# pytorch/audio

Measured on AMD Instinct MI355X. Metric: audio-sec/sec MelSpectrogram (b=256, 16kHz, n_fft=400, n_mels=80), higher is better.
Workload: dtype f32; 1 GPU; MelSpectrogram n_fft=400 hop=160 n_mels=80, batch=256 x 10 s @16 kHz fp32 per GPU (BASELINE configs[1]); per_gpu_batch=256

## Files before the change

audio_amd/csrc/melspec400.h:

```cpp
#pragma once
#include <type_traits>
#include "hd.h"
#include "stft_generic.h"
#include "resample_mfma.h"

namespace aamd {
namespace m400 {

constexpr int kN = 400;
constexpr int kPad = 200;
constexpr int kFramesPerWave = 6;
#ifndef AAMD_M400_WAVES
#define AAMD_M400_WAVES 12
#define AAMD_M400_MINWAVES 3
#endif
constexpr int kWavesPerBlock = AAMD_M400_WAVES;
constexpr int kTOff[20] = {0, 260, 520, 652, 784, 916, 1444, 1576, 128, 388,
                           2104, 2232, 2364, 1708, 1840, 1048, 1180, 1312, 1972, 2492};
constexpr int kTBufDwords = 2492 + 128;
constexpr int kTRow = 44;
constexpr int kTPair = 20 * kTRow;
constexpr int kLdsDwordsPerWave = 3 * kTPair;
constexpr int kPK = 208;
constexpr int kPPair = 416;
// ... 383 lines not shown
    if (blk >= TREG) {
#pragma unroll
      for (int j = 0; j < 10; ++j) tw[j] = twn[j];
      if (blk < 3) tw_load(blk + 1);
    } else {
#pragma unroll
      for (int j = 0; j < 10; ++j) tw[j] = twr[10 * blk + j];
    }
    float wr[5], wi[5];
#pragma unroll
    for (int j = 0; j < 5; ++j) {
      const int s = 5 * blk + j;
      if (s == 0) {
        wr[j] = yr[0];
        wi[j] = yi[0];
      } else {
        wr[j] = yr[s] * tw[2 * j] - yi[s] * tw[2 * j + 1];
        wi[j] = yr[s] * tw[2 * j + 1] + yi[s] * tw[2 * j];
      }
    }
#if defined(__HIP_DEVICE_COMPILE__)
    if (blk == 0) tr_store5<0>(lds_base, wr, wi);
    else if (blk == 1) tr_store5<5>(lds_base, wr, wi);
    else if (blk == 2) tr_store5<10>(lds_base, wr, wi);
    else tr_store5<15>(lds_base, wr, wi);
#else
    const int l = 20 * c.p + c.pi;
#pragma unroll
    for (int j = 0; j < 5; ++j) {
      lds[kTOff[5 * blk + j] + l] = wr[j];
      lds[kTOff[5 * blk + j] + 64 + l] = wi[j];
    }
#endif
  }
}

template <int H, bool WREG = false, int TREG = 0>
AAMD_HD void phase_a(const LaneConst& c, const float (&X)[Hop<H>::nx], float* lds, const float* winr = nullptr,
                     const float* twr = nullptr) {
  float xr[20], xi[20];
  if (WREG) {
#pragma unroll
    for (int q = 0; q < 20; ++q) { xr[q] = X[q] * winr[q]; xi[q] = X[q + H] * winr[q]; }
  } else {
#pragma unroll
    for (int q4 = 0; q4 < 5; ++q4) {
      const F4 w = *reinterpret_cast<const F4*>(c.win + 4 * q4);
      const float wv[4] = {w.x, w.y, w.z, w.w};
#pragma unroll
      for (int e = 0; e < 4; ++e) {
        const int q = 4 * q4 + e;
        xr[q] = X[q] * wv[e];
        xi[q] = X[q + H] * wv[e];
      }
    }
  }
  phase_a_core<TREG>(c, xr, xi, lds, twr);
}

AAMD_HD void phase_b1_load(const LaneConst& c, const float* lds, float (&vr)[20], float (&vi)[20]) {
  const float* col = lds + c.troff;
#pragma unroll
  for (int j = 0; j < 5; ++j) {
    const F4 r = *reinterpret_cast<const F4*>(col + 4 * j);
    const F4 i = *reinterpret_cast<const F4*>(col + 64 + 4 * j);
    vr[4 * j] = r.x; vr[4 * j + 1] = r.y; vr[4 * j + 2] = r.z; vr[4 * j + 3] = r.w;
    vi[4 * j] = i.x; vi[4 * j + 1] = i.y; vi[4 * j + 2] = i.z; vi[4 * j + 3] = i.w;
  }
}

AAMD_HD void phase_b2_send(const LaneConst& c, const float (&zr)[20], const float (&zi)[20],
                           float (&qr)[10], float (&qi)[10]) {
  const bool c0 = (c.col == 0);
#pragma unroll
  for (int i = 0; i < 10; ++i) {
    const int j = 10 + i;
    const float nr = zr[j], ni = zi[j], rr = zr[(j + 1) % 20], ri = zi[(j + 1) % 20];
    qr[i] = c0 ? rr : nr;
    qi[i] = c0 ? ri : ni;
  }
}

AAMD_HD void phase_b2(const LaneConst& c, const float (&zr)[20], const float (&zi)[20],
                      const float (&xr)[10], const float (&xi)[10], float* lds) {
  if (!c.active) return;
  float* P = lds + kPPair * c.p + 2 * c.col;
#pragma unroll
  for (int u = 0; u < 10; ++u) {
    const float cr = xr[9 - u], ci = xi[9 - u];
    const float ar = zr[u] + cr, ai = zi[u] - ci;
    const float br = zr[u] - cr, bi = zi[u] + ci;
    *reinterpret_cast<F2*>(P + 40 * u) = F2{ar * ar + ai * ai, br * br + bi * bi};
  }
  if (c.col == 0) {
    const float ar = zr[10] + zr[10], bi = zi[10] + zi[10];
    *reinterpret_cast<F2*>(P + 400) = F2{ar * ar, bi * bi};
  }
}

AAMD_HD float spec_pow(float m2, float power) {
  if (power == 2.0f) return m2;
  const float m = sqrt(m2);
  if (power == 1.0f) return m;
  return pow(m, power);
}

AAMD_HD void phase_b2_spec(const LaneConst& c, const float (&zr)[20], const float (&zi)[20],
                           const float (&xr)[10], const float (&xi)[10], float power, int phase, float* lds) {
  if (!c.active) return;
  float* Ra = lds + phase + kSpecBins * 2 * c.p + c.col;
  float* Rb = Ra + kSpecBins;
#pragma unroll
  for (int u = 0; u < 10; ++u) {
    const float cr = xr[9 - u], ci = xi[9 - u];
    const float ar = zr[u] + cr, ai = zi[u] - ci;
    const float br = zr[u] - cr, bi = zi[u] + ci;
    Ra[20 * u] = spec_pow(ar * ar + ai * ai, power);
    Rb[20 * u] = spec_pow(br * br + bi * bi, power);
  }
  if (c.col == 0) {
    const float ar = zr[10] + zr[10], bi = zi[10] + zi[10];
    Ra[200] = spec_pow(ar * ar, power);
    Rb[200] = spec_pow(bi * bi, power);
  }
}

AAMD_HD void phase_b2_spec_complex(const LaneConst& c, const float (&zr)[20], const float (&zi)[20],
                                   const float (&xr)[10], const float (&xi)[10], int half, int phase, float* lds) {
  if (!c.active) return;
  const int fa = 2 * c.p - 3 * half, fb = fa + 1;
  const bool wa = fa >= 0 && fa < 3, wb = fb >= 0 && fb < 3;
  float* Ra = lds + phase + 2 * kSpecBins * fa + 2 * c.col;
  float* Rb = lds + phase + 2 * kSpecBins * fb + 2 * c.col;
#pragma unroll
  for (int u = 0; u < 10; ++u) {
    const float cr = xr[9 - u], ci = xi[9 - u];
    if (wa) { Ra[40 * u] = zr[u] + cr; Ra[40 * u + 1] = zi[u] - ci; }
    if (wb) { Rb[40 * u] = zi[u] + ci; Rb[40 * u + 1] = cr - zr[u]; }
  }
  if (c.col == 0) {
    if (wa) { Ra[400] = zr[10] + zr[10]; Ra[401] = 0.0f; }
    if (wb) { Rb[400] = zi[10] + zi[10]; Rb[401] = 0.0f; }
  }
}

AAMD_HD void store_spec(int lane, const float* lds, float* out, int64_t a0, int n_floats) {
  const int phase = (int)(a0 & 3);
  float* base = out + (a0 - phase);
  const int n_pieces = (phase + n_floats + 3) >> 2;
  for (int j = lane; j < n_pieces; j += 64) {
    const int i0 = 4 * j;
    if (i0 >= phase && i0 + 4 <= phase + n_floats) {
      *reinterpret_cast<F4*>(base + i0) = *reinterpret_cast<const F4*>(lds + i0);
    } else {
      for (int e = 0; e < 4; ++e)
        if (i0 + e >= phase && i0 + e < phase + n_floats) base[i0 + e] = lds[i0 + e];
    }
  }
}

#ifndef AAMD_M400_SPEC_FULL
#define AAMD_M400_SPEC_FULL 1
#endif
AAMD_HD void store_spec_full(int lane, const float* lds, float* out, int64_t a0) {
  constexpr int kN = kFramesPerWave * kSpecBins;
  const int phase = (int)(a0 & 3);
  float* base = out + (a0 - phase);
  const int n_pieces = (phase + kN + 3) >> 2;
  F4 v[5];
#pragma unroll
  for (int u = 0; u < 5; ++u) {
    const int j = lane + 64 * u;
    if (u < 4 || j < n_pieces) v[u] = *reinterpret_cast<const F4*>(lds + 4 * j);
  }
#pragma unroll
  for (int u = 0; u < 5; ++u) {
    const int j = lane + 64 * u, i0 = 4 * j;
    const bool full = i0 >= phase && i0 + 4 <= phase + kN;
    if ((u < 4 || j < n_pieces) && full) *reinterpret_cast<F4*>(base + i0) = v[u];
  }
  if (lane == 0 && phase != 0) {
    const float e[4] = {v[0].x, v[0].y, v[0].z, v[0].w};
#pragma unroll
    for (int k = 1; k < 4; ++k)
      if (k >= phase) base[k] = e[k];
  }
  const int jl = n_pieces - 1, il = 4 * jl;
  if (lane + 256 == jl && il + 4 > phase + kN) {
    const float e[4] = {v[4].x, v[4].y, v[4].z, v[4].w};
#pragma unroll
    for (int k = 0; k < 3; ++k)
      if (il + k < phase + kN) base[il + k] = e[k];
  }
}

AAMD_HD float fast_log10(float x) {
#if defined(__HIP_DEVICE_COMPILE__)
  return __log2f(x) * 0.30102999566398120f;
#else
  return log10(x);
#endif
}
AAMD_HD float epi_plog(float x) {
  const float kE = 2.718281828459045f;
#if defined(__HIP_DEVICE_COMPILE__)
  const float lg = __log2f(x) * 0.69314718055994531f;
#else
  const float lg = log(x);
#endif
  const float t = x > kE ? lg : x;
  return t <= kE ? t / kE : t;
}
AAMD_HD float epi_db(float x, const Epi400& e) {
  return e.multiplier * fast_log10(fmax(x, e.amin)) - e.db_sub;
}

AAMD_HD void phase_b2_pad(int lane, float* lds) {
  constexpr int kTail = kPK - 201;
  if (lane < 3 * kTail) {
    const int p = lane / kTail, j = lane - p * kTail;
    *reinterpret_cast<F2*>(lds + kPPair * p + 2 * (201 + j)) = F2{0.0f, 0.0f};
  }
}

template <int NC>
AAMD_HD void mel_chunks(const float* wt, const float* P, float& sa, float& sb) {
  F4 w[NC], q0[NC], q1[NC];
#pragma unroll
  for (int k = 0; k < NC; ++k) {
    w[k] = *reinterpret_cast<const F4*>(wt + 4 * k);
    q0[k] = *reinterpret_cast<const F4*>(P + 8 * k);
    q1[k] = *reinterpret_cast<const F4*>(P + 8 * k + 4);
  }
#pragma unroll
  for (int k = 0; k < NC; ++k) {
    sa += w[k].x * q0[k].x;
    sb += w[k].x * q0[k].y;
    sa += w[k].y * q0[k].z;
    sb += w[k].y * q0[k].w;
    sa += w[k].z * q1[k].x;
    sb += w[k].z * q1[k].y;
    sa += w[k].w * q1[k].z;
    sb += w[k].w * q1[k].w;
  }
}

template <int NR>
struct MelRegs {
  int nc[NR];
  int pm[NR];
  AAMD_HD int poff(int r) const { return pm[r] & 0xffff; }
  AAMD_HD int mel(int r) const { return pm[r] >> 16; }
};

template <int NR>
AAMD_HD void mel_regs_load(const LaneConst& c, const MelTab& mt, MelRegs<NR>& h) {
#pragma unroll
  for (int r = 0; r < NR; ++r) {
    const bool on = r < mt.n_rounds;
    const int row = r * kMelSlots + c.pi;
#if defined(__HIP_DEVICE_COMPILE__)
    h.nc[r] = on ? __builtin_amdgcn_readfirstlane(mt.rc[r]) : 0;
#else
    h.nc[r] = on ? mt.rc[r] : 0;
#endif
    const int poff = on ? 2 * mt.lo2[row] : 0;
    const int mel = on ? mt.row_mel[row] : -1;
    h.pm[r] = (int)(((unsigned)mel << 16) | (unsigned)poff);
  }
}

AAMD_HD constexpr int sig_chunks(int sig, int r) { return (sig >> (4 * r)) & 15; }
constexpr int kSigHtk80 = 0x4221, kSigSlaney80 = 0x4211;

template <int NR = kMelMaxRounds, int SIG = 0, bool FENCED = false>
AAMD_HD void phase_c(const LaneConst& c, const MelTab& mt, const float* lds,
                     float (&acc_a)[NR], float (&acc_b)[NR], const MelRegs<NR>* h = nullptr) {
  const float* Pp = lds + kPPair * c.p;
  const float* wt0 = mt.w + c.pi * mt.ws;
#pragma unroll
  for (int r = 0; r < NR; ++r) {
    float sa = 0.0f, sb = 0.0f;
#if defined(__HIP_DEVICE_COMPILE__)
    if (FENCED && SIG != 0 && r > 0 && (r & 1) == 0) __builtin_amdgcn_sched_barrier(0);
#endif
    if (SIG != 0 || r < mt.n_rounds) {
      const float* wt = wt0 + r * kMelSlots * mt.ws;
      const float* P = Pp + (h ? h->poff(r) : 2 * mt.lo2[r * kMelSlots + c.pi]);
      const int nc = SIG != 0 ? sig_chunks(SIG, r) : (h ? h->nc[r] : mt.rc[r]);
      switch (nc) {
        case 1: mel_chunks<1>(wt, P, sa, sb); break;
        case 2: mel_chunks<2>(wt, P, sa, sb); break;
        case 3: mel_chunks<3>(wt, P, sa, sb); break;
        case 4: mel_chunks<4>(wt, P, sa, sb); break;
        default:
          for (int k = 0; k < nc; ++k) mel_chunks<1>(wt + 4 * k, P + 8 * k, sa, sb);
      }
    }
    acc_a[r] = sa;
    acc_b[r] = sb;
  }
}

template <int NR = kMelMaxRounds, int SIG = 0>
AAMD_HD void store_direct(const LaneConst& c, const MelTab& mt, const float (&acc_a)[NR],
                          const float (&acc_b)[NR], float* out_row, int64_t t0, int n_frames,
                          const MelRegs<NR>* h = nullptr) {
  const int left = (int)(n_frames - t0);
  const bool va = c.active && 2 * c.p < left, vb = c.active && 2 * c.p + 1 < left;
  float* out_tile = out_row + t0 * (int64_t)mt.n_mels;
  const unsigned oa = 2u * (unsigned)c.p * (unsigned)mt.n_mels;
  if (SIG != 0) {
    if (va) {
#pragma unroll
      for (int r = 0; r < NR; ++r) out_tile[oa + (unsigned)h->mel(r)] = acc_a[r];
    }
    if (vb) {
#pragma unroll
      for (int r = 0; r < NR; ++r) out_tile[oa + (unsigned)mt.n_mels + (unsigned)h->mel(r)] = acc_b[r];
    }
    return;
  }
#pragma unroll
  for (int r = 0; r < NR; ++r) {
    if (r < mt.n_rounds) {
      const int m = h ? h->mel(r) : mt.row_mel[r * kMelSlots + c.pi];
      if (m >= 0) {
        if (va) out_tile[oa + (unsigned)m] = acc_a[r];
        if (vb) out_tile[oa + (unsigned)mt.n_mels + (unsigned)m] = acc_b[r];
      }
    }
  }
}

template <int NR = kMelMaxRounds>
AAMD_HD void store_stage(const LaneConst& c, const MelTab& mt, const float (&acc_a)[NR],
                         const float (&acc_b)[NR], float* lds, const MelRegs<NR>* h = nullptr) {
  if (!c.active) return;
  float* oa = lds + 2 * c.p * mt.n_mels;
#pragma unroll
  for (int r = 0; r < NR; ++r) {
    if (r < mt.n_rounds) {
      const int m = h ? h->mel(r) : mt.row_mel[r * kMelSlots + c.pi];
      if (m >= 0) {
        oa[m] = acc_a[r];
        oa[mt.n_mels + m] = acc_b[r];
      }
    }
  }
}

AAMD_HD void store_wide(int lane, const MelTab& mt, const float* lds, float* out_row, int64_t t0,
                        int n_frames) {
  const int64_t left = n_frames - t0;
  const int n_valid = left < kFramesPerWave ? (int)left : kFramesPerWave;
  const int pieces = n_valid * mt.n_mels / 4;
  float* dst = out_row + t0 * (int64_t)mt.n_mels;
  for (int j = lane; j < pieces; j += 64)
    *reinterpret_cast<F4*>(dst + 4 * j) = *reinterpret_cast<const F4*>(lds + 4 * j);
}

#if defined(__HIPCC__)
__device__ __forceinline__ float vmax_raw(float x, float y) {
  float r;
  asm("v_max_f32 %0, %1, %2" : "=v"(r) : "v"(x), "v"(y));
  return r;
}
__device__ __forceinline__ float vmin_raw(float x, float y) {
  float r;
  asm("v_min_f32 %0, %1, %2" : "=v"(r) : "v"(x), "v"(y));
  return r;
}
__device__ __forceinline__ float vmax3_raw(float x, float y, float z) {
  float r;
  asm("v_max3_f32 %0, %1, %2, %3" : "=v"(r) : "v"(x), "v"(y), "v"(z));
  return r;
}
__device__ __forceinline__ float vmin3_raw(float x, float y, float z) {
  float r;
  asm("v_min3_f32 %0, %1, %2, %3" : "=v"(r) : "v"(x), "v"(y), "v"(z));
  return r;
}
__device__ __forceinline__ void wave_lds_fence() {
  asm volatile("" ::: "memory");
}

__device__ __forceinline__ void exchange_partner(float (&qr)[10], float (&qi)[10], unsigned long long self_mask) {
  unsigned long long saved;
  asm volatile(
      "s_mov_b64 %[sv], exec\n\t"
      "s_andn2_b64 exec, exec, %[m]\n\t"
      "s_nop 4\n\t"
      "v_mov_b32_dpp %0, %0 quad_perm:[1,0,3,2] row_mask:0xf bank_mask:0xf\n\t"
      "v_mov_b32_dpp %1, %1 quad_perm:[1,0,3,2] row_mask:0xf bank_mask:0xf\n\t"
      "v_mov_b32_dpp %2, %2 quad_perm:[1,0,3,2] row_mask:0xf bank_mask:0xf\n\t"
      "v_mov_b32_dpp %3, %3 quad_perm:[1,0,3,2] row_mask:0xf bank_mask:0xf\n\t"
      "v_mov_b32_dpp %4, %4 quad_perm:[1,0,3,2] row_mask:0xf bank_mask:0xf\n\t"
      "v_mov_b32_dpp %5, %5 quad_perm:[1,0,3,2] row_mask:0xf bank_mask:0xf\n\t"
      "v_mov_b32_dpp %6, %6 quad_perm:[1,0,3,2] row_mask:0xf bank_mask:0xf\n\t"
      "v_mov_b32_dpp %7, %7 quad_perm:[1,0,3,2] row_mask:0xf bank_mask:0xf\n\t"
      "v_mov_b32_dpp %8, %8 quad_perm:[1,0,3,2] row_mask:0xf bank_mask:0xf\n\t"
      "v_mov_b32_dpp %9, %9 quad_perm:[1,0,3,2] row_mask:0xf bank_mask:0xf\n\t"
      "v_mov_b32_dpp %10, %10 quad_perm:[1,0,3,2] row_mask:0xf bank_mask:0xf\n\t"
      "v_mov_b32_dpp %11, %11 quad_perm:[1,0,3,2] row_mask:0xf bank_mask:0xf\n\t"
      "v_mov_b32_dpp %12, %12 quad_perm:[1,0,3,2] row_mask:0xf bank_mask:0xf\n\t"
      "v_mov_b32_dpp %13, %13 quad_perm:[1,0,3,2] row_mask:0xf bank_mask:0xf\n\t"
      "v_mov_b32_dpp %14, %14 quad_perm:[1,0,3,2] row_mask:0xf bank_mask:0xf\n\t"
      "v_mov_b32_dpp %15, %15 quad_perm:[1,0,3,2] row_mask:0xf bank_mask:0xf\n\t"
      "v_mov_b32_dpp %16, %16 quad_perm:[1,0,3,2] row_mask:0xf bank_mask:0xf\n\t"
      "v_mov_b32_dpp %17, %17 quad_perm:[1,0,3,2] row_mask:0xf bank_mask:0xf\n\t"
      "v_mov_b32_dpp %18, %18 quad_perm:[1,0,3,2] row_mask:0xf bank_mask:0xf\n\t"
      "v_mov_b32_dpp %19, %19 quad_perm:[1,0,3,2] row_mask:0xf bank_mask:0xf\n\t"
      "s_mov_b64 exec, %[sv]"
      : "+v"(qr[0]), "+v"(qr[1]), "+v"(qr[2]), "+v"(qr[3]), "+v"(qr[4]), "+v"(qr[5]), "+v"(qr[6]), "+v"(qr[7]),
        "+v"(qr[8]), "+v"(qr[9]), "+v"(qi[0]), "+v"(qi[1]), "+v"(qi[2]), "+v"(qi[3]), "+v"(qi[4]), "+v"(qi[5]),
        "+v"(qi[6]), "+v"(qi[7]), "+v"(qi[8]), "+v"(qi[9]), [sv] "=&s"(saved)
      : [m] "s"(self_mask));
}

__device__ __forceinline__ void glds16(const void* gsrc, unsigned lds_dst) {
  asm volatile("s_mov_b32 m0, %1\n\ts_nop 0\n\tglobal_load_lds_dwordx4 %0, off" : : "v"(gsrc), "s"(lds_dst) : "memory", "m0");
}

#ifndef AAMD_M400_DMA_SADDR
#define AAMD_M400_DMA_SADDR 1
#endif
__device__ __forceinline__ void glds16s(const void* sbase, unsigned voff_bytes, unsigned lds_dst) {
  asm volatile("s_mov_b32 m0, %2\n\ts_nop 0\n\tglobal_load_lds_dwordx4 %0, %1" : : "v"(voff_bytes), "s"(sbase), "s"(lds_dst) : "memory", "m0");
}
__device__ __forceinline__ void stage_wait() { asm volatile("s_waitcnt vmcnt(0)" ::: "memory"); }

struct TileInfo {
  int64_t row, t0;
  bool staged;
};

__device__ __forceinline__ void atomic_max_f32(float* addr, float v) {
  if (v >= 0.0f) atomicMax(reinterpret_cast<int*>(addr), __float_as_int(v));
  else atomicMin(reinterpret_cast<unsigned int*>(addr), __float_as_uint(v));
}

__global__ void __launch_bounds__(256) mfcc_frag_build_kernel(const float* __restrict__ dct, int n_mels, int n_mfcc,
                                                              float* __restrict__ frag) {
  uint16_t* fh = reinterpret_cast<uint16_t*>(frag);
  const int n = kMfccMT * kMfccSteps * 64 * 8;
  for (int i = blockIdx.x * blockDim.x + threadIdx.x; i < n; i += gridDim.x * blockDim.x) {
    const int j = i & 7, lane = (i >> 3) & 63, g = i >> 9, s = g % kMfccSteps, t = g / kMfccSteps;
    const float v = mfcc_frag_value(dct, n_mels, n_mfcc, t, s, lane, j);
    const uint16_t hi = rsm::f16_bits(v);
    const uint16_t lo = rsm::f16_bits(v - rsm::f16_value(hi));
    fh[mfcc_frag_piece(t, s, 0, lane) * 8 + j] = hi;
    fh[mfcc_frag_piece(t, s, 1, lane) * 8 + j] = lo;
  }
}

__global__ void __launch_bounds__(256) mel_tab_build_kernel(MelBandsDev mb, float* __restrict__ out) {
  MelTab mt{};
  mel_tab_rounds(threadIdx.x, blockDim.x, mb, out, mt);
  __syncthreads();
  mel_tab_fill(threadIdx.x, blockDim.x, mb, out, mt);
}

template <int LAB, int EPI, int H = 8, typename TIn = float, int NR = kMelMaxRounds, int SIG = 0>
__global__ void __launch_bounds__(64 * kWavesPerBlock, AAMD_M400_MINWAVES)
melspec400_kernel(const TIn* __restrict__ wav, const float* __restrict__ window,
                  const float* __restrict__ tw400, MelBandsDev mb, float* __restrict__ out,
                  int64_t rows, int64_t length, int64_t row_stride, int n_frames, float scale,
                  int tiles_per_row, int64_t n_tiles, int tiles_per_block, int in_aligned,
                  int out_wide, Epi400 epi) {
  extern __shared__ __attribute__((aligned(16))) float smem400[];
  unsigned fix_base = 0, fix_cnt = 0;
#if defined(AAMD_LAB) && defined(AAMD_MFCC_FIXUP_RETURNS)
  if (EPI == EPI400_MFCC && epi.fixup != 0) return;
#endif
  if (EPI == EPI400_MFCC && epi.fixup != 0) {
    int* const cnt = reinterpret_cast<int*>(smem400);
    if (threadIdx.x == 0) *cnt = 0;
    __syncthreads();
    const unsigned nt = (unsigned)n_tiles, nbk = gridDim.x, b = blockIdx.x;
    const unsigned n_cand = b < nt ? (nt - b + nbk - 1u) / nbk : 0u;
    fix_base = b * (nt / nbk) + (b < nt % nbk ? b : nt % nbk);
    for (unsigned k0 = 0; k0 < n_cand; k0 += blockDim.x) {
      const unsigned k = k0 + threadIdx.x;
      bool hit = false;
      unsigned t = 0;
      if (k < n_cand) {
        t = b + k * nbk;
        const unsigned row = t / (unsigned)tiles_per_row;
        hit = epi.tile_min[t] < epi.group_max[row / epi.rows_per_group] - epi.top_db;
      }
      const unsigned long long m = __ballot(hit);
      int slot = 0;
      if ((threadIdx.x & 63) == 0 && m)
        slot = __hip_atomic_fetch_add(cnt, __popcll(m), __ATOMIC_RELAXED, __HIP_MEMORY_SCOPE_WORKGROUP);
      slot = __builtin_amdgcn_readfirstlane(slot);
      if (hit) epi.fix_list[fix_base + slot + __popcll(m & ((1ull << (threadIdx.x & 63)) - 1ull))] = (int)t;
    }
    __syncthreads();
    fix_cnt = (unsigned)__builtin_amdgcn_readfirstlane(*cnt);
    if (fix_cnt == 0) return;
    if (threadIdx.x == 0) atomicAdd(epi.fix_count, (int)fix_cnt);
    __syncthreads();
  }
  if (EPI == EPI400_MFCC && epi.fixup == 0 && epi.fix_count != nullptr && !(LAB & (1048576 | 8388608)) && blockIdx.x == 0 &&
      threadIdx.x == 0)
    *epi.fix_count = 0;
  const int elab = (LAB & 524288) ? epi.lab : 0;
  const int lane = threadIdx.x & 63;
  const int wave = __builtin_amdgcn_readfirstlane(threadIdx.x >> 6);
#ifdef AAMD_M400_PRIO
  {
    const int pr = AAMD_M400_PRIO == 1 ? (wave >> 2) : AAMD_M400_PRIO == 2 ? 2 - (wave >> 2) : (wave >> 2) == 0 ? 1 : 0;
    if (pr == 1) __builtin_amdgcn_s_setprio(1);
    else if (pr == 2) __builtin_amdgcn_s_setprio(2);
  }
#endif
  long long lab_t0 = 0;
  if (LAB & 1024) lab_t0 = wall_clock64();
  if ((LAB & 1048576) && lane == 0) {
    long long* rec = reinterpret_cast<long long*>(epi.fix_count);
    const int w = blockIdx.x * kWavesPerBlock + wave;
    rec[4 * w] = (long long)clock64();
    rec[4 * w + 1] = wall_clock64();
  }
  using HC = Hop<H>;
  constexpr int kHop = HC::hop;
  float* lds = smem400 + wave * HC::lds_dwords;
  const unsigned s_addr = (unsigned)(uintptr_t)(lds + kSOff);

  float* const_tab = smem400 + kWavesPerBlock * HC::lds_dwords;
  const_tab_build(threadIdx.x, blockDim.x, window, tw400, scale, const_tab);
  MelTab mt{};
  const int tab_dwords = (EPI != EPI400_SPEC) ? mel_tab_dwords(mb.n_mels, mb.max_width) : 0;
  int* queue = reinterpret_cast<int*>(const_tab + kConstDwords + tab_dwords);
  constexpr bool kIoWave = (LAB & 16777216) != 0;
  constexpr int kNio = kIoWave ? ((LAB & 67108864) ? 2 : 1) : 0;
  if (threadIdx.x == 0) *queue = kWavesPerBlock - kNio;
  float* frag_lds = const_tab + kConstDwords + tab_dwords + 4;
  constexpr bool kFragLds = (H != 10);
  if (EPI == EPI400_MFCC && (epi.frag_in_lds != 0) != kFragLds) __builtin_trap();
  if (EPI == EPI400_MFCC && kFragLds)
    for (int i = threadIdx.x; i < kMfccFragFloats; i += blockDim.x) frag_lds[i] = epi.dct_frag[i];
  if (EPI != EPI400_SPEC && mb.table400 != nullptr) {
    float* dst = const_tab + kConstDwords;
    for (int i = threadIdx.x; i < tab_dwords; i += blockDim.x) dst[i] = mb.table400[i];
    mel_tab_layout(mb, dst, mt);
    __syncthreads();
  } else {
    if (EPI != EPI400_SPEC) mel_tab_rounds(threadIdx.x, blockDim.x, mb, const_tab + kConstDwords, mt);
    __syncthreads();
    if (EPI != EPI400_SPEC) mel_tab_fill(threadIdx.x, blockDim.x, mb, const_tab + kConstDwords, mt);
    __syncthreads();
  }

  long long lab_t1 = 0;
  if (LAB & 1024) lab_t1 = wall_clock64();
  LaneConst c;
  lane_init(lane, const_tab, c);
  constexpr bool kWinRegs = (EPI != EPI400_MFCC || H != 10) && (((LAB & 8192) != 0) || !(LAB & 262144));
  float winr[20], twr[40];
  if (kWinRegs) {
#pragma unroll
    for (int q = 0; q < 20; ++q) winr[q] = c.win[q];
  }
#ifndef AAMD_M400_TWREG
#define AAMD_M400_TWREG 3
#endif
#ifndef AAMD_M400_TWREG_DB
#define AAMD_M400_TWREG_DB 1
#endif
#ifndef AAMD_M400_TWREG_MFCC
#define AAMD_M400_TWREG_MFCC 2
#endif
  constexpr bool kPlain = H == 8 && std::is_same<TIn, float>::value && LAB == 0;
  constexpr int kTwRegBatches = (LAB & 16384) ? 4
                                : (SIG != 0 && EPI == EPI400_MEL) ? AAMD_M400_TWREG
                                : !kPlain ? 0
                                : EPI == EPI400_SPEC ? 2
                                : (EPI == EPI400_MEL && SIG == 0) ? (NR <= 4 ? 1 : 3)
                                : (EPI == EPI400_MFCC && NR <= 4) ? AAMD_M400_TWREG_MFCC
                                : (EPI == EPI400_MEL_DB && NR <= 4) ? AAMD_M400_TWREG_DB : 0;
  if (kTwRegBatches > 0) {
#pragma unroll
    for (int q = 0; q < 10 * kTwRegBatches; ++q) twr[q] = c.tw[q];
  }
  constexpr bool kHoist = NR <= 4;
  MelRegs<NR> mregs;
  const MelRegs<NR>* mh = nullptr;
  if (EPI != EPI400_SPEC && kHoist) {
    mel_regs_load<NR>(c, mt, mregs);
    mh = &mregs;
  }
  if (SIG != 0) {
    static_assert(SIG == 0 || NR == 4, "filterbank signatures are 4 rounds of 20 mels");
    const int sig_rt = mregs.nc[0] | (mregs.nc[1 % NR] << 4) | (mregs.nc[2 % NR] << 8) | (mregs.nc[3 % NR] << 12);
    if (mt.n_rounds != NR || mt.n_mels != kMelSlots * NR || sig_rt != SIG) __builtin_trap();
  }
  if (EPI == EPI400_MFCC && (mt.n_rounds != NR || mt.n_mels != kMelSlots * NR)) __builtin_trap();
  float nrm_mean[NR], nrm_inv[NR];
  if (EPI == EPI400_MEL_NORM) {
#pragma unroll
    for (int r = 0; r < NR; ++r) {
      const int m = r < mt.n_rounds ? mt.row_mel[r * kMelSlots + c.pi] : -1;
      nrm_mean[r] = m >= 0 ? epi.mean[m] : 0.0f;
      nrm_inv[r] = m >= 0 ? epi.invstd[m] : 0.0f;
    }
  }
  const unsigned long long self_mask = __ballot((c.col == 0) || (c.col == 10));
  using SG = Stage<H, TIn>;
  static_assert(SG::ok, "no staging layout for this hop / input type");
  int spiece[SG::ndma];
#pragma unroll
  for (int k = 0; k < SG::ndma; ++k) spiece[k] = SG::spp * stage_src_piece<H, TIn>(64 * k + lane);

  const int nb = gridDim.x;
  int lb = blockIdx.x;
  if ((nb & 7) == 0) lb = (blockIdx.x & 7) * (nb >> 3) + (blockIdx.x >> 3);
  unsigned blk_first = (unsigned)lb * (unsigned)tiles_per_block;
  unsigned blk_count = 0;
  if (blk_first < (unsigned)n_tiles) {
    blk_count = (unsigned)n_tiles - blk_first;
    if (blk_count > (unsigned)tiles_per_block) blk_count = (unsigned)tiles_per_block;
  }
  if (EPI == EPI400_MFCC && epi.fixup != 0) {
    blk_first = 0;
    blk_count = fix_cnt;
  }
  auto claim = [&]() {
    int v = 0;
    if (lane == 0) v = __hip_atomic_fetch_add(queue, 1, __ATOMIC_RELAXED, __HIP_MEMORY_SCOPE_WORKGROUP);
    return (unsigned)__builtin_amdgcn_readfirstlane(v);
  };
#if AAMD_M400_POOLS
#define AAMD_M400_POOLED (AAMD_M400_POOLS && (LAB == 0) && epi.pool != nullptr && !(EPI == EPI400_MFCC && epi.fixup != 0))
  if (AAMD_M400_POOLED && blk_count > (unsigned)(tiles_per_block - epi.pool_p)) blk_count = (unsigned)(tiles_per_block - epi.pool_p);
  unsigned pool_ticket = 0;
  auto pool_request = [&]() {
    int lbo = (int)(blk_first / (unsigned)tiles_per_block);
    asm volatile("" : "+s"(lbo));
    unsigned* const ctr = epi.pool + (lbo % pool_count(nb)) * kPoolStride;
    if (lane == 0) pool_ticket = __hip_atomic_fetch_add(ctr, 1u, __ATOMIC_RELAXED, __HIP_MEMORY_SCOPE_AGENT);
  };
  auto pool_take = [&]() {
    int lbo = (int)(blk_first / (unsigned)tiles_per_block);
    asm volatile("" : "+s"(lbo));
    const int np = pool_count(nb), pid = lbo % np, mem = pool_members(nb, np, pid);
    for (;;) {
      const unsigned v = (unsigned)__builtin_amdgcn_readfirstlane((int)pool_ticket);
      if (v + 1u == (unsigned)(mem * (epi.pool_p + kWavesPerBlock)) && lane == 0)
        __hip_atomic_store(epi.pool + pid * kPoolStride, 0u, __ATOMIC_RELAXED, __HIP_MEMORY_SCOPE_AGENT);
      bool exhausted;
      const unsigned t = pool_tile(np, epi.pool_p, tiles_per_block, (unsigned)n_tiles, pid, mem, v, exhausted);
      if (t != kNoTile) return t - blk_first;
      if (exhausted) return 0x80000000u;
      pool_request();
    }
  };
  constexpr unsigned kBadIdx = 0x80000000u, kPendIdx = 0x80000001u;
#define AAMD_M400_IDX_OK(I) ((((I) ^ 0x80000000u)) > 1u)
#define AAMD_M400_LOCAL(I) ((I) < blk_count ? (I) : kBadIdx)
#else
#define AAMD_M400_IDX_OK(I) ((I) < blk_count)
#define AAMD_M400_LOCAL(I) (I)
#endif
  constexpr unsigned kLabChunk = 8;
  unsigned* gq = reinterpret_cast<unsigned*>(epi.group_max);
  int g_pending = 0;
  unsigned g_base = 0, g_pos = 0;
  auto g_request = [&]() {
    if (lane == 0) g_pending = (int)__hip_atomic_fetch_add(gq, 1u, __ATOMIC_RELAXED, __HIP_MEMORY_SCOPE_AGENT);
  };
  if (LAB & 131072) {
    blk_count = (unsigned)n_tiles;
    g_request();
    g_base = (unsigned)__builtin_amdgcn_readfirstlane(g_pending) * kLabChunk;
    g_request();
  }
  auto g_next = [&]() {
    if (++g_pos < kLabChunk) return g_base + g_pos;
    g_base = (unsigned)__builtin_amdgcn_readfirstlane(g_pending) * kLabChunk;
    g_pos = 0;
    g_request();
    return g_base;
  };

  auto tile_info = [&](unsigned idx) {
    TileInfo ti;
    unsigned t = ((LAB & 131072) ? 0u : blk_first) + idx;
    if (EPI == EPI400_MFCC && epi.fixup != 0)
      t = idx < blk_count ? (unsigned)__hip_atomic_load(epi.fix_list + fix_base + idx, __ATOMIC_RELAXED, __HIP_MEMORY_SCOPE_AGENT) : 0u;
    const unsigned row = t / (unsigned)tiles_per_row;
    ti.row = row;
    ti.t0 = (int64_t)(t - row * (unsigned)tiles_per_row) * kFramesPerWave;
    ti.staged = AAMD_M400_IDX_OK(idx) && in_aligned && (ti.t0 * kHop - kPad >= 0) &&
                ((ti.t0 + kFramesPerWave - 1) * kHop + (kN - kPad) <= length) &&
                (ti.t0 + kFramesPerWave <= n_frames);
    return ti;
  };
  auto stage_issue = [&](const TileInfo& ti) {
    const TIn* src = wav + (ti.row / InTraits<TIn>::chans) * row_stride + (ti.t0 * kHop - kPad);
    if (LAB & 32) src = wav + 6 * kHop;
#pragma unroll
    for (int k = 0; k < SG::ndma; ++k)
      if (!(LAB & 64) || k == 0) {
#if AAMD_M400_DMA_SADDR
        glds16s(src, (unsigned)spiece[k] * (unsigned)sizeof(TIn), s_addr + 1024 * k);
#else
        glds16(src + spiece[k], s_addr + 1024 * k);
#endif
      }
  };

  float wmax = -INFINITY;
  int64_t wgroup = -1, wrow = -1;
  constexpr bool kDb = (EPI == EPI400_MEL_DB) || (EPI == EPI400_MFCC);
  const bool fix = (EPI == EPI400_MFCC) && epi.fixup != 0;
  auto flush_max = [&]() {
    if (kDb && !fix && epi.group_max != nullptr && wgroup >= 0) {
      float m = wmax;
#pragma unroll
      for (int off = 32; off > 0; off >>= 1) m = fmaxf(m, __shfl_xor(m, off, 64));
      if (lane == 0) atomic_max_f32(epi.group_max + wgroup, m);
    }
    wmax = -INFINITY;
  };

  if (kIoWave && wave >= kWavesPerBlock - kNio) {
    constexpr unsigned D = 8;
    constexpr bool kFetchOnly = (LAB & 134217728) != 0;
    if (!(LAB & 33554432)) {
      const unsigned n_mine = (blk_count + (unsigned)kNio - 1u - (unsigned)(wave - (kWavesPerBlock - kNio))) / (unsigned)kNio;
      for (unsigned i = 0; i < n_mine + D; ++i) {
        const unsigned t = i * (unsigned)kNio + (unsigned)(wave - (kWavesPerBlock - kNio));
        if (i < n_mine) {
          const TileInfo ti = tile_info(AAMD_M400_LOCAL(t));
          const unsigned dst = (unsigned)(uintptr_t)(smem400 + (t % (unsigned)kWavesPerBlock) * HC::lds_dwords + kSOff);
          if (ti.staged) {
            const TIn* src = wav + (ti.row / InTraits<TIn>::chans) * row_stride + (ti.t0 * kHop - kPad);
#pragma unroll
            for (int k = 0; k < SG::ndma; ++k) glds16(src + spiece[k], dst + 1024 * k);
          }
        }
        if (i >= D) {
          if (kFetchOnly) {
            asm volatile("s_waitcnt vmcnt(40)" ::: "memory");
          } else {
            asm volatile("s_waitcnt vmcnt(56)" ::: "memory");
            const unsigned told = t - D * (unsigned)kNio;
            const TileInfo to = tile_info(AAMD_M400_LOCAL(told));
            const float* stg = smem400 + (told % (unsigned)kWavesPerBlock) * HC::lds_dwords;
            store_wide(lane, mt, stg, out + to.row * (int64_t)n_frames * (int64_t)mb.n_mels, to.t0, n_frames);
          }
        }
      }
    }
    blk_count = 0;
  }
  unsigned cur_idx = (LAB & 131072) ? g_base : (unsigned)wave;
#if AAMD_M400_POOLS
  if (cur_idx >= blk_count) cur_idx = kBadIdx;
  if (AAMD_M400_POOLED && cur_idx == kBadIdx) {
    pool_request();
    cur_idx = pool_take();
  }
#endif
  TileInfo cur = tile_info(cur_idx);
  if (LAB & 128) {
    const int k = (wave + 6 * lb) % 3;
    for (int i = 0; i < k; ++i) __builtin_amdgcn_s_sleep(112);
  }
  if (LAB & 2048) {
    const int k = 4 * (wave & 3) + (wave >> 2) % 3;
    for (int i = 0; i < (k % 12); ++i) __builtin_amdgcn_s_sleep(17);
  }
  if (LAB & 4096) {
    const int k = 4 * ((wave >> 2) % 3) + (wave & 3);
    for (int i = 0; i < k; ++i) __builtin_amdgcn_s_sleep(17);
  }
  float Xn[HC::nx];
  auto gload = [&](const TileInfo& ti) {
    const TIn* src = wav + (ti.row / InTraits<TIn>::chans) * row_stride + (ti.t0 * kHop - kPad) + (HC::pair_stride * c.p + c.pi);
#pragma unroll
    for (int q = 0; q < HC::nx; ++q) Xn[q] = InTraits<TIn>::get(src + 20 * q, (int)(ti.row % InTraits<TIn>::chans));
  };
  if (LAB & 32768) {
#pragma unroll
    for (int q = 0; q < HC::nx; ++q) Xn[q] = 0.0f;
    if (cur.staged) gload(cur);
  } else if (cur.staged && !(LAB & 8) && !fix) {
    stage_issue(cur);
  }

  long long ph_acc[6] = {0, 0, 0, 0, 0, 0}, ph_t = 0;
  int ph_tiles = 0;
#define AAMD_M400_STAMP(K)                                  \
  if (LAB & 8388608) {                                      \
    const long long now_ = (long long)clock64();            \
    ph_acc[K] += now_ - ph_t;                               \
    ph_t = now_;                                            \
  }
  using mfcc_f32x4 = __attribute__((ext_vector_type(4))) float;
  mfcc_f32x4 cf[kMfccMT];
  const int mfcc_elab = (LAB & 524288) ? epi.lab : 0;
  auto mfcc_finish = [&](int64_t row, int64_t t0) {
#pragma unroll
    for (int t = 0; t < kMfccMT; ++t)
#pragma unroll
      for (int i = 0; i < 4; ++i) {
        cf[t][i] += __int_as_float(__builtin_amdgcn_mov_dpp(__float_as_int(cf[t][i]), 0x128, 0xf, 0xf, true));
        asm volatile("" : "+v"(cf[t][i]));
      }
    const int64_t left64 = n_frames - t0;
    const int left = left64 < kFramesPerWave ? (int)left64 : kFramesPerWave;
    if (!(LAB & 2) && !(mfcc_elab & 8) && (lane & 15) < left) {
      float* otile = out + (row * (int64_t)n_frames + t0) * (int64_t)epi.n_mfcc;
      const unsigned ooff = (unsigned)(lane & 15) * (unsigned)epi.n_mfcc + 4u * (unsigned)(lane >> 4);
#pragma unroll
      for (int t = 0; t < kMfccMT; ++t) {
        const int k0 = 16 * t + 4 * (lane >> 4);
        if (k0 < epi.n_mfcc) *reinterpret_cast<F4*>(otile + (ooff + 16u * (unsigned)t)) = F4{cf[t][0], cf[t][1], cf[t][2], cf[t][3]};
      }
    }
  };
  while (AAMD_M400_IDX_OK(cur_idx)) {
    if (LAB & 8388608) { ph_t = (long long)clock64(); ++ph_tiles; }
#if AAMD_M400_POOLS
    unsigned nxt_idx = (LAB & 131072) ? g_next() : claim();
    if (nxt_idx >= blk_count) nxt_idx = AAMD_M400_POOLED ? kPendIdx : kBadIdx;
#else
    const unsigned nxt_idx = (LAB & 131072) ? g_next() : claim();
#endif
    TileInfo nxt = tile_info(nxt_idx);
    float fix_cut = -INFINITY;
    if (fix) {
      fix_cut = epi.group_max[cur.row / epi.rows_per_group] - epi.top_db;
      if (cur.staged) stage_issue(cur);
    }

    float X[HC::nx];
    if ((LAB & 32768) && cur.staged) {
#pragma unroll
      for (int q = 0; q < HC::nx; ++q) X[q] = Xn[q];
    } else if (cur.staged) {
      if (!(LAB & 1)) stage_wait();
      if (LAB & 256) {
#pragma unroll
        for (int q = 0; q < HC::nx; ++q) X[q] = (float)(q + lane) * scale;
      } else {
        gather_lds<H, TIn>(c, reinterpret_cast<const TIn*>(lds + kSOff), X, (int)(cur.row % InTraits<TIn>::chans));
      }
    } else {
      gather_global<H, TIn>(c, wav + (cur.row / InTraits<TIn>::chans) * row_stride, length, cur.t0, n_frames, X,
                            (int)(cur.row % InTraits<TIn>::chans));
    }
#if AAMD_M400_POOLS
    if (nxt_idx == kPendIdx) pool_request();
#endif
    phase_a<H, kWinRegs, kTwRegBatches>(c, X, lds, winr, twr);
    if ((LAB & 32768) && nxt.staged) gload(nxt);
    wave_lds_fence();
    AAMD_M400_STAMP(0)
    float vr[20], vi[20], zr[20], zi[20], qr[10], qi[10];
    phase_b1_load(c, lds, vr, vi);
    if (!(LAB & 32768)) {
      asm volatile("s_waitcnt lgkmcnt(0)" ::: "memory");
      AAMD_M400_STAMP(1)
#if AAMD_M400_POOLS
      if (nxt_idx == kPendIdx) {
        nxt_idx = pool_take();
        nxt = tile_info(nxt_idx);
      }
#endif
      if (nxt.staged && !(LAB & 8) && !fix) stage_issue(nxt);
    }
    if (LAB & 16) { wave_lds_fence(); cur = nxt; cur_idx = nxt_idx; continue; }
    dft20(vr, vi, zr, zi);
    phase_b2_send(c, zr, zi, qr, qi);
    exchange_partner(qr, qi, self_mask);
    wave_lds_fence();
    AAMD_M400_STAMP(2)
    if (EPI == EPI400_SPEC) {
      const int64_t left = n_frames - cur.t0;
      const int n_valid = left < kFramesPerWave ? (int)left : kFramesPerWave;
      if (epi.power > 0.0f) {
        const int64_t a0 = (cur.row * n_frames + cur.t0) * (int64_t)kSpecBins;
        phase_b2_spec(c, zr, zi, qr, qi, epi.power, (int)(a0 & 3), lds);
        wave_lds_fence();
        if (!(LAB & 2)) {
          if (AAMD_M400_SPEC_FULL && n_valid == kFramesPerWave) store_spec_full(lane, lds, out, a0);
          else store_spec(lane, lds, out, a0, n_valid * kSpecBins);
        }
        wave_lds_fence();
      } else {
#pragma unroll
        for (int half = 0; half < 2; ++half) {
          const int64_t a0 = (cur.row * n_frames + cur.t0 + 3 * half) * (int64_t)(2 * kSpecBins);
          const int nv = n_valid - 3 * half < 3 ? n_valid - 3 * half : 3;
          phase_b2_spec_complex(c, zr, zi, qr, qi, half, (int)(a0 & 3), lds);
          wave_lds_fence();
          if (!(LAB & 2) && nv > 0) store_spec(lane, lds, out, a0, nv * 2 * kSpecBins);
          wave_lds_fence();
        }
      }
      cur = nxt;
      cur_idx = nxt_idx;
      continue;
    }
    phase_b2(c, zr, zi, qr, qi, lds);
    phase_b2_pad(lane, lds);
    wave_lds_fence();
    AAMD_M400_STAMP(3)
    float acc_a[NR], acc_b[NR];
    if (LAB & 4) { wave_lds_fence(); cur = nxt; cur_idx = nxt_idx; continue; }
    phase_c<NR, SIG, EPI == EPI400_MFCC>(c, mt, lds, acc_a, acc_b, mh);
    if (LAB & 8388608) { asm volatile("" : "+v"(acc_a[0]), "+v"(acc_b[NR - 1])); }
    AAMD_M400_STAMP(4)
    if (kDb) {
      if (cur.row != wrow) {
        wrow = cur.row;
        const int64_t g = cur.row / epi.rows_per_group;
        if (g != wgroup) {
          flush_max();
          wgroup = g;
        }
      }
      const bool va_ok = cur.t0 + 2 * c.p < n_frames, vb_ok = cur.t0 + 2 * c.p + 1 < n_frames;
      float tmin = INFINITY;
      if (EPI == EPI400_MFCC) {
        const float db_c1 = epi.multiplier * 0.30102999566398120f;
#pragma unroll
        for (int r = 0; r < NR; ++r) {
          acc_a[r] = __builtin_fmaf(__log2f(vmax_raw(acc_a[r], epi.amin)), db_c1, -epi.db_sub);
          acc_b[r] = __builtin_fmaf(__log2f(vmax_raw(acc_b[r], epi.amin)), db_c1, -epi.db_sub);
        }
        if (cur.t0 + kFramesPerWave <= n_frames) {
#pragma unroll
          for (int r = 0; r < NR; ++r) {
            wmax = vmax3_raw(wmax, acc_a[r], acc_b[r]);
            tmin = vmin3_raw(tmin, acc_a[r], acc_b[r]);
          }
        } else {
#pragma unroll
          for (int r = 0; r < NR; ++r) {
            wmax = fmaxf(wmax, fmaxf(va_ok ? acc_a[r] : -INFINITY, vb_ok ? acc_b[r] : -INFINITY));
            tmin = fminf(tmin, fminf(va_ok ? acc_a[r] : INFINITY, vb_ok ? acc_b[r] : INFINITY));
          }
        }
        if (fix) {
#pragma unroll
          for (int r = 0; r < NR; ++r) {
            acc_a[r] = vmax_raw(acc_a[r], fix_cut);
            acc_b[r] = vmax_raw(acc_b[r], fix_cut);
          }
        }
      } else {
        const bool interior = cur.t0 + kFramesPerWave <= n_frames;
#pragma unroll
        for (int r = 0; r < NR; ++r) {
          if (r < mt.n_rounds) {
            acc_a[r] = epi.multiplier * fast_log10(vmax_raw(acc_a[r], epi.amin)) - epi.db_sub;
            acc_b[r] = epi.multiplier * fast_log10(vmax_raw(acc_b[r], epi.amin)) - epi.db_sub;
            if (interior) wmax = vmax3_raw(wmax, acc_a[r], acc_b[r]);
            else wmax = fmaxf(wmax, fmaxf(va_ok ? acc_a[r] : -INFINITY, vb_ok ? acc_b[r] : -INFINITY));
          }
        }
      }
      if (EPI == EPI400_MFCC && !fix && !(elab & 4)) {
        asm volatile(
            "s_nop 1\n\t"
            "v_min_f32_dpp %0, %0, %0 row_shr:1 row_mask:0xf bank_mask:0xf\n\ts_nop 1\n\t"
            "v_min_f32_dpp %0, %0, %0 row_shr:2 row_mask:0xf bank_mask:0xf\n\ts_nop 1\n\t"
            "v_min_f32_dpp %0, %0, %0 row_shr:4 row_mask:0xf bank_mask:0xf\n\ts_nop 1\n\t"
            "v_min_f32_dpp %0, %0, %0 row_shr:8 row_mask:0xf bank_mask:0xf\n\ts_nop 1\n\t"
            "v_min_f32_dpp %0, %0, %0 row_bcast:15 row_mask:0xa bank_mask:0xf\n\ts_nop 1\n\t"
            "v_min_f32_dpp %0, %0, %0 row_bcast:31 row_mask:0xc bank_mask:0xf"
            : "+v"(tmin));
        if (lane == 63) epi.tile_min[blk_first + cur_idx] = tmin;
      }
    }
    if (EPI == EPI400_MFCC) {
      using f32x4 = __attribute__((ext_vector_type(4))) float;
      using h8 = __attribute__((ext_vector_type(8))) _Float16;
      using h4 = __attribute__((ext_vector_type(4))) _Float16;
      using u32x4 = __attribute__((ext_vector_type(4))) uint32_t;
      using u32x2 = __attribute__((ext_vector_type(2))) uint32_t;
      wave_lds_fence();
      {
        uint16_t* hs = reinterpret_cast<uint16_t*>(lds);
        uint16_t* ls = hs + kMfccPlaneHalves;
#pragma unroll
        for (int r = 0; r < NR; ++r) {
          const int m = mh ? mh->mel(r) : mt.row_mel[r * kMelSlots + c.pi];
          const float va = acc_a[r] * kMfccYScale, vb = acc_b[r] * kMfccYScale;
          const _Float16 ha = (_Float16)va, hb = (_Float16)vb;
          const _Float16 la = (_Float16)(va - (float)ha), lb = (_Float16)(vb - (float)hb);
          hs[2 * c.p * kMfccMels + m] = __builtin_bit_cast(uint16_t, ha);
          ls[2 * c.p * kMfccMels + m] = __builtin_bit_cast(uint16_t, la);
          hs[(2 * c.p + 1) * kMfccMels + m] = __builtin_bit_cast(uint16_t, hb);
          ls[(2 * c.p + 1) * kMfccMels + m] = __builtin_bit_cast(uint16_t, lb);
        }
      }
      wave_lds_fence();
#pragma unroll
      for (int t = 0; t < kMfccMT; ++t) cf[t] = f32x4{0.0f, 0.0f, 0.0f, 0.0f};
      auto product = [&](const u32x4* __restrict__ ftab) {
        const uint16_t* hs = reinterpret_cast<const uint16_t*>(lds);
        u32x4 a0[kMfccMT][2];
        auto frag_load = [&](int sidx) {
#pragma unroll
          for (int t = 0; t < kMfccMT; ++t)
#pragma unroll
            for (int hl = 0; hl < 2; ++hl) {
              a0[t][hl] = u32x4{0x3c003c00u, 0x3c003c00u, 0x3c003c00u, 0x3c003c00u};
              if (!(elab & 1)) a0[t][hl] = ftab[mfcc_frag_piece(t, sidx, hl, lane)];
            }
        };
#pragma unroll
        for (int sidx = 0; sidx < 2; ++sidx) {
          const h8 bb = __builtin_bit_cast(h8, *reinterpret_cast<const u32x4*>(hs + mfcc_b_index(lane, sidx)));
          frag_load(sidx);
#pragma unroll
          for (int t = 0; t < kMfccMT; ++t)
            cf[t] = __builtin_amdgcn_mfma_f32_16x16x32_f16(__builtin_bit_cast(h8, a0[t][1]), bb, cf[t], 0, 0, 0);
#pragma unroll
          for (int t = 0; t < kMfccMT; ++t)
            cf[t] = __builtin_amdgcn_mfma_f32_16x16x32_f16(__builtin_bit_cast(h8, a0[t][0]), bb, cf[t], 0, 0, 0);
        }
        {
          frag_load(2);
          const h4 bb = __builtin_bit_cast(h4, *reinterpret_cast<const u32x2*>(hs + mfcc_b_index(lane, 2)));
#define AAMD_A4(T, HL) __builtin_bit_cast(h4, u32x2{a0[T][HL][0], a0[T][HL][1]})
#pragma unroll
          for (int t = 0; t < kMfccMT; ++t) cf[t] = __builtin_amdgcn_mfma_f32_16x16x16f16(AAMD_A4(t, 1), bb, cf[t], 0, 0, 0);
#pragma unroll
          for (int t = 0; t < kMfccMT; ++t) cf[t] = __builtin_amdgcn_mfma_f32_16x16x16f16(AAMD_A4(t, 0), bb, cf[t], 0, 0, 0);
#undef AAMD_A4
        }
      };
      if (!(elab & 2)) {
        if (kFragLds) product(reinterpret_cast<const u32x4*>(frag_lds));
        else product(reinterpret_cast<const u32x4*>(epi.dct_frag));
      }
      if (!(elab & 2)) mfcc_finish(cur.row, cur.t0);
      wave_lds_fence();
      cur = nxt;
      cur_idx = nxt_idx;
      continue;
    }
    if (EPI == EPI400_MEL_NORM) {
#pragma unroll
      for (int r = 0; r < NR; ++r) {
        if (r < mt.n_rounds) {
          acc_a[r] = (epi_plog(acc_a[r] * epi.gain) - nrm_mean[r]) * nrm_inv[r];
          acc_b[r] = (epi_plog(acc_b[r] * epi.gain) - nrm_mean[r]) * nrm_inv[r];
        }
      }
    }
    float* out_row = out + cur.row * (EPI == EPI400_MEL_NORM ? epi.out_frames : (int64_t)n_frames) * (int64_t)mb.n_mels;
    if (LAB & 4194304) out_row = out + (int64_t)(wave + kWavesPerBlock * (blockIdx.x & 63)) * 6 * mb.n_mels - cur.t0 * (int64_t)mb.n_mels;
    if (out_wide) {
      wave_lds_fence();
      store_stage<NR>(c, mt, acc_a, acc_b, lds, mh);
      wave_lds_fence();
      if (!(LAB & 2)) store_wide(lane, mt, lds, out_row, cur.t0, n_frames);
    } else {
      if (!(LAB & 2)) store_direct<NR, SIG>(c, mt, acc_a, acc_b, out_row, cur.t0, n_frames, mh);
    }
    wave_lds_fence();
    AAMD_M400_STAMP(5)
    cur = nxt;
    cur_idx = nxt_idx;
  }
#undef AAMD_M400_STAMP
  if ((LAB & 8388608) && lane == 0) {
    long long* rec = reinterpret_cast<long long*>(epi.fix_count) + 4 * 12 * 256 + 8 * (blockIdx.x * kWavesPerBlock + wave);
#pragma unroll
    for (int k = 0; k < 6; ++k) rec[k] = ph_acc[k];
    rec[6] = ph_tiles;
  }
  if (kDb && !fix && epi.group_max != nullptr) {
    float m = wmax;
#pragma unroll
    for (int off = 32; off > 0; off >>= 1) m = fmaxf(m, __shfl_xor(m, off, 64));
    if (lane == 0) {
      reinterpret_cast<int*>(lds)[0] = (int)wgroup;
      lds[1] = m;
    }
    __syncthreads();
    if (threadIdx.x == 0) {
      int g_run = -1;
      float m_run = -INFINITY;
      for (int w = 0; w < kWavesPerBlock; ++w) {
        const int gw = reinterpret_cast<const int*>(smem400 + w * HC::lds_dwords)[0];
        const float mw = smem400[w * HC::lds_dwords + 1];
        if (gw != g_run) {
          if (g_run >= 0) atomic_max_f32(epi.group_max + g_run, m_run);
          g_run = gw;
          m_run = mw;
        } else {
          m_run = fmaxf(m_run, mw);
        }
      }
      if (g_run >= 0) atomic_max_f32(epi.group_max + g_run, m_run);
    }
  }
  if ((LAB & 1048576) && lane == 0) {
    long long* rec = reinterpret_cast<long long*>(epi.fix_count);
    const int w = blockIdx.x * kWavesPerBlock + wave;
    rec[4 * w + 2] = (long long)clock64();
    rec[4 * w + 3] = wall_clock64();
  }
  if ((LAB & 1024) && lane == 0) {
    long long* rec = reinterpret_cast<long long*>(const_cast<float*>(tw400) + 1024);
    const int w = blockIdx.x * kWavesPerBlock + wave;
    rec[3 * w] = lab_t0;
    rec[3 * w + 1] = lab_t1;
    rec[3 * w + 2] = wall_clock64();
  }
}
#endif

}
}
```

Measured before the change: 37.47 million audio-sec/sec.

## Cut per-tile scalar address math: carry tile offsets, saddr stores, LDS queue claim

Precomputes per-tile input/output offsets in TileInfo and advances them incrementally from the previous tile instead of recomputing divisions and 64-bit multiplies. The staged-tile test is simplified to a precomputed tile-index range. Mel output stores use global_store_dword with a scalar base and immediate offsets, with a fast path for full tiles. The tile-queue claim uses an inline ds_add_rtn in place of the HIP atomic. This targets the integer and address overhead in the persistent tile loop. It adds inline asm and carry logic that must stay consistent with the tile indexing.

```diff
diff --git a/audio_amd/csrc/melspec400.h b/audio_amd/csrc/melspec400.h
--- a/audio_amd/csrc/melspec400.h
+++ b/audio_amd/csrc/melspec400.h
@@ -709,6 +709,15 @@
   }
 }
 
+template <int OFF>
+AAMD_HD void store_f32_saddr(float v, char* base, unsigned voff) {
+#if defined(__HIP_DEVICE_COMPILE__)
+  asm volatile("global_store_dword %0, %1, %2 offset:%3" : : "v"(voff), "v"(v), "s"(base), "i"(OFF) : "memory");
+#else
+  *reinterpret_cast<float*>(base + (size_t)voff + OFF) = v;
+#endif
+}
+
 template <int NR = kMelMaxRounds, int SIG = 0>
 AAMD_HD void store_direct(const LaneConst& c, const MelTab& mt, const float (&acc_a)[NR],
                           const float (&acc_b)[NR], float* out_row, int64_t t0, int n_frames,
@@ -718,13 +727,27 @@
   float* out_tile = out_row + t0 * (int64_t)mt.n_mels;
   const unsigned oa = 2u * (unsigned)c.p * (unsigned)mt.n_mels;
   if (SIG != 0) {
+    constexpr unsigned nm = kMelSlots * NR;
+    char* const ob = reinterpret_cast<char*>(out_row + t0 * (int64_t)nm);
+    unsigned bo[NR];
+#pragma unroll
+    for (int r = 0; r < NR; ++r) bo[r] = 4u * (2u * (unsigned)c.p * nm + (unsigned)h->mel(r));
+    if (left >= kFramesPerWave) {
+      if (c.active) {
+#pragma unroll
+        for (int r = 0; r < NR; ++r) store_f32_saddr<0>(acc_a[r], ob, bo[r]);
+#pragma unroll
+        for (int r = 0; r < NR; ++r) store_f32_saddr<4 * (int)nm>(acc_b[r], ob, bo[r]);
+      }
+      return;
+    }
     if (va) {
 #pragma unroll
-      for (int r = 0; r < NR; ++r) out_tile[oa + (unsigned)h->mel(r)] = acc_a[r];
+      for (int r = 0; r < NR; ++r) store_f32_saddr<0>(acc_a[r], ob, bo[r]);
     }
     if (vb) {
 #pragma unroll
-      for (int r = 0; r < NR; ++r) out_tile[oa + (unsigned)mt.n_mels + (unsigned)h->mel(r)] = acc_b[r];
+      for (int r = 0; r < NR; ++r) store_f32_saddr<4 * (int)nm>(acc_b[r], ob, bo[r]);
     }
     return;
   }
@@ -838,8 +861,12 @@
 __device__ __forceinline__ void stage_wait() { asm volatile("s_waitcnt vmcnt(0)" ::: "memory"); }
 
 struct TileInfo {
-  int64_t row, t0;
+  int64_t row;
+  int t0;
   bool staged;
+  unsigned tin;
+  int64_t in_off;
+  int64_t out_off;
 };
 
 __device__ __forceinline__ void atomic_max_f32(float* addr, float v) {
@@ -1033,9 +1060,11 @@
     blk_first = 0;
     blk_count = fix_cnt;
   }
+  const unsigned queue_addr = (unsigned)(uintptr_t)queue;
   auto claim = [&]() {
     int v = 0;
-    if (lane == 0) v = __hip_atomic_fetch_add(queue, 1, __ATOMIC_RELAXED, __HIP_MEMORY_SCOPE_WORKGROUP);
+    if (lane == 0)
+      asm volatile("ds_add_rtn_u32 %0, %1, %2\n\ts_waitcnt lgkmcnt(0)" : "=v"(v) : "v"(queue_addr), "v"(1) : "memory");
     return (unsigned)__builtin_amdgcn_readfirstlane(v);
   };
 #if AAMD_M400_POOLS
@@ -1091,6 +1120,21 @@
     return g_base;
   };
 
+  static_assert(kFramesPerWave * kHop >= kPad, "tile 1 starts inside the clip");
+  unsigned tin_hi = 0;
+  if (in_aligned && length >= kN - kPad) {
+    int64_t last = (length - (kN - kPad)) / kHop - (kFramesPerWave - 1);
+    if (last > (int64_t)n_frames - kFramesPerWave) last = (int64_t)n_frames - kFramesPerWave;
+    if (last >= kFramesPerWave) tin_hi = (unsigned)(last / kFramesPerWave);
+  }
+  const int64_t out_row_elems =
+      EPI == EPI400_SPEC   ? (int64_t)n_frames * (epi.power > 0.0f ? kSpecBins : 2 * kSpecBins)
+      : EPI == EPI400_MFCC ? (int64_t)n_frames * epi.n_mfcc
+                           : (EPI == EPI400_MEL_NORM ? epi.out_frames : (int64_t)n_frames) * (int64_t)mb.n_mels;
+  auto tile_fill = [&](TileInfo& ti, unsigned idx) {
+    ti.t0 = (int)ti.tin * kFramesPerWave;
+    ti.staged = AAMD_M400_IDX_OK(idx) && ti.tin - 1u < tin_hi;
+  };
   auto tile_info = [&](unsigned idx) {
     TileInfo ti;
     unsigned t = ((LAB & 131072) ? 0u : blk_first) + idx;
@@ -1098,14 +1142,33 @@
       t = idx < blk_count ? (unsigned)__hip_atomic_load(epi.fix_list + fix_base + idx, __ATOMIC_RELAXED, __HIP_MEMORY_SCOPE_AGENT) : 0u;
     const unsigned row = t / (unsigned)tiles_per_row;
     ti.row = row;
-    ti.t0 = (int64_t)(t - row * (unsigned)tiles_per_row) * kFramesPerWave;
-    ti.staged = AAMD_M400_IDX_OK(idx) && in_aligned && (ti.t0 * kHop - kPad >= 0) &&
-                ((ti.t0 + kFramesPerWave - 1) * kHop + (kN - kPad) <= length) &&
-                (ti.t0 + kFramesPerWave <= n_frames);
+    ti.tin = t - row * (unsigned)tiles_per_row;
+    ti.in_off = (ti.row / InTraits<TIn>::chans) * row_stride;
+    ti.out_off = ti.row * out_row_elems;
+    tile_fill(ti, idx);
+    return ti;
+  };
+  constexpr bool kCarry = !(LAB & (131072 | 16777216)) && !AAMD_M400_POOLS && EPI != EPI400_MFCC && InTraits<TIn>::chans == 1;
+  constexpr unsigned kCarryMinTiles = 16;
+  auto tile_next = [&](const TileInfo& from, unsigned from_idx, unsigned idx) {
+    if (!kCarry || (unsigned)tiles_per_row < kCarryMinTiles) return tile_info(idx);
+    TileInfo ti = from;
+    if (!(AAMD_M400_IDX_OK(idx))) {
+      ti.staged = false;
+      return ti;
+    }
+    ti.tin = from.tin + (idx - from_idx);
+    while (ti.tin >= (unsigned)tiles_per_row) {
+      ti.tin -= (unsigned)tiles_per_row;
+      ti.row += 1;
+      ti.in_off += row_stride;
+      ti.out_off += out_row_elems;
+    }
+    tile_fill(ti, idx);
     return ti;
   };
   auto stage_issue = [&](const TileInfo& ti) {
-    const TIn* src = wav + (ti.row / InTraits<TIn>::chans) * row_stride + (ti.t0 * kHop - kPad);
+    const TIn* src = wav + ti.in_off + ((int64_t)ti.t0 * kHop - kPad);
     if (LAB & 32) src = wav + 6 * kHop;
 #pragma unroll
     for (int k = 0; k < SG::ndma; ++k)
@@ -1143,7 +1206,7 @@
           const TileInfo ti = tile_info(AAMD_M400_LOCAL(t));
           const unsigned dst = (unsigned)(uintptr_t)(smem400 + (t % (unsigned)kWavesPerBlock) * HC::lds_dwords + kSOff);
           if (ti.staged) {
-            const TIn* src = wav + (ti.row / InTraits<TIn>::chans) * row_stride + (ti.t0 * kHop - kPad);
+            const TIn* src = wav + ti.in_off + ((int64_t)ti.t0 * kHop - kPad);
 #pragma unroll
             for (int k = 0; k < SG::ndma; ++k) glds16(src + spiece[k], dst + 1024 * k);
           }
@@ -1186,7 +1249,7 @@
   }
   float Xn[HC::nx];
   auto gload = [&](const TileInfo& ti) {
-    const TIn* src = wav + (ti.row / InTraits<TIn>::chans) * row_stride + (ti.t0 * kHop - kPad) + (HC::pair_stride * c.p + c.pi);
+    const TIn* src = wav + ti.in_off + ((int64_t)ti.t0 * kHop - kPad) + (HC::pair_stride * c.p + c.pi);
 #pragma unroll
     for (int q = 0; q < HC::nx; ++q) Xn[q] = InTraits<TIn>::get(src + 20 * q, (int)(ti.row % InTraits<TIn>::chans));
   };
@@ -1237,7 +1300,7 @@
 #else
     const unsigned nxt_idx = (LAB & 131072) ? g_next() : claim();
 #endif
-    TileInfo nxt = tile_info(nxt_idx);
+    TileInfo nxt = tile_next(cur, cur_idx, nxt_idx);
     float fix_cut = -INFINITY;
     if (fix) {
       fix_cut = epi.group_max[cur.row / epi.rows_per_group] - epi.top_db;
@@ -1257,7 +1320,7 @@
         gather_lds<H, TIn>(c, reinterpret_cast<const TIn*>(lds + kSOff), X, (int)(cur.row % InTraits<TIn>::chans));
       }
     } else {
-      gather_global<H, TIn>(c, wav + (cur.row / InTraits<TIn>::chans) * row_stride, length, cur.t0, n_frames, X,
+      gather_global<H, TIn>(c, wav + cur.in_off, length, cur.t0, n_frames, X,
                             (int)(cur.row % InTraits<TIn>::chans));
     }
 #if AAMD_M400_POOLS
@@ -1290,7 +1353,7 @@
       const int64_t left = n_frames - cur.t0;
       const int n_valid = left < kFramesPerWave ? (int)left : kFramesPerWave;
       if (epi.power > 0.0f) {
-        const int64_t a0 = (cur.row * n_frames + cur.t0) * (int64_t)kSpecBins;
+        const int64_t a0 = cur.out_off + (int64_t)cur.t0 * kSpecBins;
         phase_b2_spec(c, zr, zi, qr, qi, epi.power, (int)(a0 & 3), lds);
         wave_lds_fence();
         if (!(LAB & 2)) {
@@ -1301,7 +1364,7 @@
       } else {
 #pragma unroll
         for (int half = 0; half < 2; ++half) {
-          const int64_t a0 = (cur.row * n_frames + cur.t0 + 3 * half) * (int64_t)(2 * kSpecBins);
+          const int64_t a0 = cur.out_off + (int64_t)(cur.t0 + 3 * half) * (2 * kSpecBins);
           const int nv = n_valid - 3 * half < 3 ? n_valid - 3 * half : 3;
           phase_b2_spec_complex(c, zr, zi, qr, qi, half, (int)(a0 & 3), lds);
           wave_lds_fence();
@@ -1463,7 +1526,7 @@
         }
       }
     }
-    float* out_row = out + cur.row * (EPI == EPI400_MEL_NORM ? epi.out_frames : (int64_t)n_frames) * (int64_t)mb.n_mels;
+    float* out_row = out + cur.out_off;
     if (LAB & 4194304) out_row = out + (int64_t)(wave + kWavesPerBlock * (blockIdx.x & 63)) * 6 * mb.n_mels - cur.t0 * (int64_t)mb.n_mels;
     if (out_wide) {
       wave_lds_fence();
```

Result: faster. 38.04 million audio-sec/sec, median of 6 (+1.5%).
